# data61/stellar-random-walk

Measured on AMD Instinct MI355X. Metric: walk-steps/sec, higher is better.
Workload: dtype f64

## Files before the change

### stellar-random-walk_amd/csrc/sampler_tables.hip

```cpp
#include <cstring>

#include "engine.h"
#include "sampling.h"

namespace srw {
namespace {

constexpr int SMALL_DEG = 32;

__device__ inline bool weight_regular(float w) { return w >= 0.0f; }

struct FoStore {
  FoEnt *fo;
  __device__ inline void put(int64_t e, double cdf, int32_t id) const {
    FoEnt f; f.cdf = cdf; f.id = id; f.guide = 0; f.noff = 0; f.ndeg = 0; f.nflags = 0; fo[e] = f;
  }
  __device__ inline double cdf(int64_t e) const { return fo[e].cdf; }
  __device__ inline void set_guide(int64_t e, int32_t g) const { fo[e].guide = g; }
  __device__ inline int32_t guide(int64_t e) const { return fo[e].guide; }
};
struct SlimStore {
  double *c; int32_t *g;
  __device__ inline void put(int64_t e, double cdf, int32_t) const { c[e] = cdf; }
  __device__ inline double cdf(int64_t e) const { return c[e]; }
  __device__ inline void set_guide(int64_t e, int32_t gg) const { g[e] = gg; }
  __device__ inline int32_t guide(int64_t e) const { return g[e]; }
};

template <class ST>
__global__ void k_fo_small(Row *rows, const Ent *__restrict__ ent, ST st, int64_t n_slots) {
  for (int64_t v = blockIdx.x * (int64_t)blockDim.x + threadIdx.x; v < n_slots; v += (int64_t)gridDim.x * blockDim.x) {
    Row r = rows[v];
    if (r.deg <= 0 || r.deg > SMALL_DEG) continue;
    const Ent *row = ent + r.off;
    double sum = 0.0;
    bool irr = false;
    for (int32_t k = 0; k < r.deg; ++k) {
      float w = row[k].w;
      sum = sum + (double)w;
      irr |= !weight_regular(w);
    }
    irr |= !(sum > 0.0) || isinf(sum);
    double acc = 0.0;
    for (int32_t k = 0; k < r.deg; ++k) {
      Ent e = row[k];
      acc += (double)e.w / sum;
      st.put(r.off + k, acc, e.id);
    }
    if (irr) rows[v].flags = r.flags | ROW_IRREGULAR;
  }
}

template <class ST>
__global__ void k_fo_large(Row *rows, const Ent *__restrict__ ent, ST st, int64_t n_slots,
                           unsigned long long *next_slot) {
  const int lane = lane_id();
  while (true) {
    unsigned long long grab = 0;
    if (lane == 0) grab = atomicAdd(next_slot, 4ull);
    grab = ((unsigned long long)(uint32_t)__builtin_amdgcn_readfirstlane((int)(grab >> 32)) << 32) |
           (uint32_t)__builtin_amdgcn_readfirstlane((int)(uint32_t)grab);
    if ((int64_t)grab >= n_slots) break;
   for (int64_t v = (int64_t)grab; v < (int64_t)grab + 4 && v < n_slots; ++v) {
    Row r = rows[v];
    if (r.deg <= SMALL_DEG) continue;
    const Ent *row = ent + r.off;
    double part = 0.0;
    SumCert cert;
    bool irr = false;
    for (int32_t base = 0; base < r.deg; base += 256) {
      float wv[4]; bool ok[4];
#pragma unroll
      for (int u = 0; u < 4; ++u) {
        int32_t k = base + u * 64 + lane;
        ok[u] = k < r.deg;
        wv[u] = row[ok[u] ? k : r.deg - 1].w;
      }
#pragma unroll
      for (int u = 0; u < 4; ++u)
        if (ok[u]) { part += (double)wv[u]; cert.add(wv[u]); irr |= !weight_regular(wv[u]); }
    }
    int emin = wave_min_i32(cert.emin), emax = wave_max_i32(cert.emax);
    bool bad = __any(cert.bad);
    irr = __any(irr);
    double S;
    if (sum_is_exact(emin, emax, bad, r.deg)) {
      S = wave_sum_f64(part);
    } else {
      S = 0.0;
      for (int32_t base = 0; base < r.deg; base += 64) {
        int32_t k = base + lane;
        double wd = (k < r.deg) ? (double)row[k].w : 0.0;
        int cnt = min(64, r.deg - base);
        for (int i = 0; i < cnt; ++i) S = S + readlane_f64(wd, i);
      }
    }
    irr |= !(S > 0.0) || isinf(S);
    double acc = 0.0;
    Ent z; z.id = 0; z.w = 0.0f;
    Ent cur[4], nxt[4];
#pragma unroll
    for (int u = 0; u < 4; ++u) { int32_t k = u * 64 + lane; cur[u] = k < r.deg ? row[k] : z; }
    for (int32_t base = 0; base < r.deg; base += 256) {
#pragma unroll
      for (int u = 0; u < 4; ++u) { int64_t k = (int64_t)base + 256 + u * 64 + lane; nxt[u] = k < r.deg ? row[k] : z; }
#pragma unroll
      for (int u = 0; u < 4; ++u) {
        const int32_t cb = base + u * 64;
        if (cb < r.deg) {
          const int32_t k = cb + lane;
          const Ent e = cur[u];
          const double d = (k < r.deg) ? (double)e.w / S : 0.0;
          const int cnt = min(64, r.deg - cb);
          double mine = 0.0;
          if (cnt == 64) {
#pragma unroll
            for (int i = 0; i < 64; ++i) {
              acc = acc + readlane_f64(d, i);
              if (lane == i) mine = acc;
            }
          } else {
            for (int i = 0; i < cnt; ++i) {
              acc = acc + readlane_f64(d, i);
              if (lane == i) mine = acc;
            }
          }
          if (k < r.deg) st.put(r.off + k, mine, e.id);
        }
      }
#pragma unroll
      for (int u = 0; u < 4; ++u) cur[u] = nxt[u];
    }
    if (irr && lane == 0) rows[v].flags = r.flags | ROW_IRREGULAR;
   }
  }
}

__device__ inline double bucket_threshold(uint32_t j, uint32_t deg) {
  uint64_t m = (((uint64_t)j << 24) + deg - 1) / deg;
  return (double)m * (1.0 / 16777216.0);
}

template <class ST>
__global__ void k_guide_small(const Row *__restrict__ rows, ST st, int64_t n_slots) {
  for (int64_t v = blockIdx.x * (int64_t)blockDim.x + threadIdx.x; v < n_slots; v += (int64_t)gridDim.x * blockDim.x) {
    Row r = rows[v];
    if (r.deg <= 0 || r.deg > SMALL_DEG || (r.flags & ROW_IRREGULAR)) continue;
    int32_t k = 0;
    for (int32_t j = 0; j < r.deg; ++j) {
      double t = bucket_threshold((uint32_t)j, (uint32_t)r.deg);
      while (k < r.deg && !(st.cdf(r.off + k) >= t)) ++k;
      st.set_guide(r.off + j, k);
    }
  }
}

constexpr int GUIDE_ITEM = 8192;
struct GuideItem { uint32_t slot_lo, slot_hi_part; };

__global__ void k_guide_make_items(const Row *__restrict__ rows, int64_t n_slots, unsigned long long *counter,
                                   uint2 *__restrict__ items, unsigned long long cap) {
  for (int64_t v = blockIdx.x * (int64_t)blockDim.x + threadIdx.x; v < n_slots; v += (int64_t)gridDim.x * blockDim.x) {
    Row r = rows[v];
    if (r.deg <= SMALL_DEG || (r.flags & ROW_IRREGULAR)) continue;
    unsigned n = (unsigned)((r.deg + GUIDE_ITEM - 1) / GUIDE_ITEM);
    unsigned long long b = atomicAdd(counter, (unsigned long long)n);
    for (unsigned i = 0; i < n && b + i < cap; ++i) items[b + i] = make_uint2((uint32_t)v, ((uint32_t)(v >> 32) << 24) | i);
  }
}

template <class ST>
__device__ inline int32_t lower_bound_cdf(const ST &st, int64_t off, int32_t lo, int32_t hi, double t) {
  while (lo < hi) {
    int32_t mid = lo + ((hi - lo) >> 1);
    if (st.cdf(off + mid) >= t) hi = mid; else lo = mid + 1;
  }
  return lo;
}

template <class ST>
__global__ void k_guide_large(const Row *__restrict__ rows, ST st, const uint2 *__restrict__ items,
                              const unsigned long long *n_items_p) {
  const int lane = lane_id();
  const unsigned long long n_items = *n_items_p;
  unsigned long long wave = (blockIdx.x * (unsigned long long)blockDim.x + threadIdx.x) >> 6;
  const unsigned long long n_waves = ((unsigned long long)gridDim.x * blockDim.x) >> 6;
  for (unsigned long long it = wave; it < n_items; it += n_waves) {
    uint2 item = items[it];
    const int64_t v = (int64_t)item.x | ((int64_t)(item.y >> 24) << 32);
    const int32_t part = (int32_t)(item.y & 0xFFFFFFu);
    Row r = rows[v];
    const int32_t jb = part * GUIDE_ITEM, je = min(r.deg, jb + GUIDE_ITEM);
    int32_t start = -1;
    for (int32_t j0 = jb; j0 < je; j0 += 64) {
      const int32_t j = j0 + lane;
      int32_t ans = r.deg;
      if (j < je) {
        const double t = bucket_threshold((uint32_t)j, (uint32_t)r.deg);
        if (start < 0) {
          ans = lower_bound_cdf(st, r.off, 0, r.deg, t);
        } else {
          int32_t lo = start, step = 1;
          while (lo + step < r.deg && !(st.cdf(r.off + lo + step - 1) >= t)) { lo += step; step <<= 1; }
          ans = lower_bound_cdf(st, r.off, lo, min(r.deg, lo + step), t);
        }
        st.set_guide(r.off + j, ans);
      }
      const int last = min(63, je - j0 - 1);
      start = __builtin_amdgcn_readlane(ans, last);
    }
  }
}

__global__ void k_fo_link(const Row *__restrict__ rows, FoEnt *__restrict__ fo, int64_t n_entries, int32_t vmin,
                          int64_t n_slots) {
  for (int64_t e = blockIdx.x * (int64_t)blockDim.x + threadIdx.x; e < n_entries; e += (int64_t)gridDim.x * blockDim.x) {
    int64_t s = (int64_t)fo[e].id - vmin;
    Row r; r.off = 0; r.deg = 0; r.flags = 0;
    if (s >= 0 && s < n_slots) r = rows[s];
    fo[e].noff = r.off; fo[e].ndeg = r.deg; fo[e].nflags = r.flags;
  }
}

template <class ST>
__device__ inline void cfo_write(const ST &st, const Row *__restrict__ rows , const Ent *__restrict__ ent, int32_t vmin,
                                 int64_t n_slots, const Row &r, int32_t j, bool regular, CfoEnt *__restrict__ cfo,
                                 unsigned long long *escapes) {
  const int64_t e = r.off + j;
  const int32_t id = ent[e].id;
  const int64_t s = (int64_t)id - vmin;
  Row nr; nr.off = 0; nr.deg = 0; nr.flags = 0;
  if (s >= 0 && s < n_slots) nr = rows[s];
  bool esc = nr.deg > (int32_t)CFO_NDEG_MAX || nr.off >= ((int64_t)1 << 36);
  uint32_t cg = 0; uint32_t dbits = 0;
  if (regular) {
    const double sc = st.cdf(e) * 16777216.0;
    const uint32_t c = sc >= 16777215.0 ? 16777215u : (uint32_t)sc;
    const int32_t delta = j - st.guide(e);
    const int32_t d12 = (delta < -2047 || delta > 2047) ? CFO_GD_SAT : delta;
    dbits = (uint32_t)d12 & 0xFFFu;
    cg = c | ((dbits & 0xFFu) << 24);
  }
  CfoEnt o;
  o.cg = cg; o.id = id;
  o.link = ((uint64_t)nr.off & CFO_NOFF_MASK) | ((uint64_t)(dbits >> 8) << 36) |
           ((uint64_t)(uint32_t)min(nr.deg, (int32_t)CFO_NDEG_MAX) << 40) | ((uint64_t)((nr.flags & ROW_IRREGULAR) != 0) << 63);
  cfo[e] = o;
  if (esc) atomicAdd(escapes, 1ull);
}
template <class ST>
__global__ void k_cfo_rows(const Row *__restrict__ rows, const Row *__restrict__ link_rows, const Ent *__restrict__ ent, ST st,
                           CfoEnt *__restrict__ cfo, int64_t n_slots, int32_t vmin, unsigned long long *escapes,
                           unsigned long long *next_slot) {
  const int lane = lane_id();
  while (true) {
    unsigned long long grab = 0;
    if (lane == 0) grab = atomicAdd(next_slot, 4ull);
    grab = ((unsigned long long)(uint32_t)__builtin_amdgcn_readfirstlane((int)(grab >> 32)) << 32) |
           (uint32_t)__builtin_amdgcn_readfirstlane((int)(uint32_t)grab);
    if ((int64_t)grab >= n_slots) break;
    for (int64_t v = (int64_t)grab; v < (int64_t)grab + 4 && v < n_slots; ++v) {
      const Row r = rows[v];
      const bool regular = !(r.flags & ROW_IRREGULAR);
      for (int32_t j = lane; j < r.deg; j += 64) cfo_write(st, link_rows, ent, vmin, n_slots, r, j, regular, cfo, escapes);
    }
  }
}
__global__ void k_fo_from_slim(const Row *__restrict__ rows, const Ent *__restrict__ ent, const double *__restrict__ c,
                               const int32_t *__restrict__ g, FoEnt *__restrict__ fo, int64_t n_entries, int32_t vmin,
                               int64_t n_slots) {
  for (int64_t e = blockIdx.x * (int64_t)blockDim.x + threadIdx.x; e < n_entries; e += (int64_t)gridDim.x * blockDim.x) {
    FoEnt f; f.cdf = c[e]; f.id = ent[e].id; f.guide = g[e];
    int64_t s = (int64_t)f.id - vmin;
    Row r; r.off = 0; r.deg = 0; r.flags = 0;
    if (s >= 0 && s < n_slots) r = rows[s];
    f.noff = r.off; f.ndeg = r.deg; f.nflags = r.flags;
    fo[e] = f;
  }
}

struct PqCert {
  int emin; bool bad; double mass;
  int glsb;
  float maxv;
  __device__ PqCert() : emin(1 << 20), bad(false), mass(0.0), glsb(1 << 20), maxv(0.0f) {}
  __device__ inline void add(float x) {
    uint32_t b = __float_as_uint(x);
    int ex = (int)((b >> 23) & 0xFFu);
    if (ex == 255 || (b >> 31 && (b & 0x7FFFFFFFu))) { bad = true; return; }
    if ((b & 0x7FFFFFFFu) == 0u) return;
    int e = ex ? ex - 127 : -126;
    emin = min(emin, e);
    const uint32_t mant = (b & 0x7FFFFFu) | (ex ? 0x800000u : 0u);
    glsb = min(glsb, e - 23 + (int)__builtin_ctz(mant));
  }
  __device__ inline void add_entry(float w, float p, float q) {
    const float a = div_exact(w, q), c = div_exact(w, p);
    add(w); add(a); add(c);
    const float mx = fmaxf(w, fmaxf(a, c));
    mass += (double)mx;
    maxv = fmaxf(maxv, mx);
  }
};
__device__ inline bool pq_row_f32(int glsb, double mass) {
  if (glsb > (1 << 19) || glsb < -1000) return false;
  return mass < ldexp(1.0, 22 + glsb);
}
__device__ inline uint32_t pq_row_u16_bits(int glsb, float maxv) {
  if (glsb > 100 || glsb < -100 || !(maxv > 0.0f)) return 0u;
  const double upc = ldexp((double)maxv, -glsb);
  uint32_t c = 0;
  while (c < 7u && upc * (double)(1u << (c + 6u)) <= 65535.0) ++c;
  return (c << ROW_U16_SHIFT) | (((uint32_t)(glsb + 128) & 0xFFu) << ROW_G_SHIFT);
}
__device__ inline bool pq_row_ok(int emin, bool bad, double mass) {
  if (bad) return false;
  if (emin > (1 << 19)) return false;
  return mass <= ldexp(1.0, 51 + emin - 23);
}

__global__ void k_pq_small(Row *__restrict__ rows, const Ent *__restrict__ ent, double *__restrict__ pq,
                           uint8_t *__restrict__ ok, int64_t n_slots, float p, float q, unsigned long long *bad_rows) {
  for (int64_t v = blockIdx.x * (int64_t)blockDim.x + threadIdx.x; v < n_slots; v += (int64_t)gridDim.x * blockDim.x) {
    Row r = rows[v];
    ok[v] = 0;
    if (r.flags & ROW_PQ_BITS) { r.flags &= ~ROW_PQ_BITS; rows[v].flags = r.flags; }
    if (r.deg <= 0 || r.deg > SMALL_DEG) continue;
    PqCert c;
    for (int32_t k = 0; k < r.deg; ++k) c.add_entry(ent[r.off + k].w, p, q);
    if (!pq_row_ok(c.emin, c.bad, c.mass)) { atomicAdd(bad_rows, 1ull); continue; }
    double acc = 0.0;
    if (pq) for (int32_t k = 0; k < r.deg; ++k) { acc += (double)div_exact(ent[r.off + k].w, q); pq[r.off + k] = acc; }
    ok[v] = 1;
    rows[v].flags = r.flags | ROW_PQ_OK | (pq_row_f32(c.glsb, c.mass) ? ROW_PQ_F32 : 0u) | pq_row_u16_bits(c.glsb, c.maxv);
  }
}

__global__ void k_pq_large(Row *__restrict__ rows, const Ent *__restrict__ ent, double *__restrict__ pq,
                           uint8_t *__restrict__ ok, int64_t n_slots, float p, float q, unsigned long long *next_slot) {
  const int lane = lane_id();
  while (true) {
    unsigned long long grab = 0;
    if (lane == 0) grab = atomicAdd(next_slot, 4ull);
    grab = ((unsigned long long)(uint32_t)__builtin_amdgcn_readfirstlane((int)(grab >> 32)) << 32) |
           (uint32_t)__builtin_amdgcn_readfirstlane((int)(uint32_t)grab);
    if ((int64_t)grab >= n_slots) break;
    for (int64_t v = (int64_t)grab; v < (int64_t)grab + 4 && v < n_slots; ++v) {
      Row r = rows[v];
      if (r.deg <= SMALL_DEG) continue;
      const Ent *row = ent + r.off;
      PqCert c;
      for (int32_t k = lane; k < r.deg; k += 64) c.add_entry(row[k].w, p, q);
      const int emin = wave_min_i32(c.emin), glsb = wave_min_i32(c.glsb);
      const bool bad = __any(c.bad);
      const double mass = wave_sum_f64(bad ? 0.0 : c.mass);
      const float maxv = __int_as_float(wave_max_i32(__float_as_int(bad ? 0.0f : c.maxv)));
      if (!pq_row_ok(emin, bad, mass)) { if (lane == 0) atomicAdd(next_slot + 1, 1ull); continue; }
      double carry = 0.0;
      for (int32_t base = 0; base < r.deg; base += 64) {
        int32_t k = base + lane;
        double x = k < r.deg ? (double)div_exact(row[k].w, q) : 0.0;
        for (int o = 1; o < 64; o <<= 1) { double t = __shfl_up(x, o); if (lane >= o) x += t; }
        if (pq && k < r.deg) pq[r.off + k] = carry + x;
        carry += readlane_f64(x, 63);
      }
      if (lane == 0) { ok[v] = 1; rows[v].flags = r.flags | ROW_PQ_OK | (pq_row_f32(glsb, mass) ? ROW_PQ_F32 : 0u) | pq_row_u16_bits(glsb, maxv); }
    }
  }
}

}

void build_pq_tables(srw_handle *h, float p, float q) {
  Graph &g = h->g;
  uint32_t pb, qb; memcpy(&pb, &p, 4); memcpy(&qb, &q, 4);
  if (g.has_pq && g.pq_pbits == pb && g.pq_qbits == qb) return;
  hipStream_t st = h->stream;
  g.has_pq = false;
  size_t free_b = 0, total_b = 0;
  SRW_HIP(hipMemGetInfo(&free_b, &total_b));
  const bool unit = !getenv("SRW_NO_UNIT_PQ") && graph_has_unit_weights(h);
  g.pq_unit = unit ? (double)(1.0f / q) : 0.0;
  const size_t need = (unit ? 0 : (size_t)g.n_entries * sizeof(double)) + (size_t)g.n_slots;
  if (!unit && g.pq.n < (size_t)g.n_entries && free_b < need + ((size_t)8 << 30)) return;
  if (unit) g.pq.release(); else g.pq.ensure((size_t)g.n_entries);
  g.pq_ok.ensure((size_t)g.n_slots);
  int gs = (int)std::min<int64_t>(std::max<int64_t>((g.n_slots + 255) / 256, 1), 256 * 32);
  DevBuf<unsigned long long> next_slot; next_slot.alloc(2);
  SRW_HIP(hipMemsetAsync(next_slot.p, 0, 16, st));
  hipLaunchKernelGGL(k_pq_small, dim3(gs), dim3(256), 0, st, g.rows.p, g.ent.p, g.pq.p, g.pq_ok.p, g.n_slots, p, q, next_slot.p + 1);
  hipLaunchKernelGGL(k_pq_large, dim3(256 * 8), dim3(256), 0, st, g.rows.p, g.ent.p, g.pq.p, g.pq_ok.p, g.n_slots, p, q,
                     next_slot.p);
  SRW_HIP(hipGetLastError());
  unsigned long long nbad = 0;
  SRW_HIP(hipMemcpyAsync(&nbad, next_slot.p + 1, 8, hipMemcpyDeviceToHost, st));
  SRW_HIP(hipStreamSynchronize(st));
  g.pq_bad_rows = (int64_t)nbad;
  g.pq_pbits = pb; g.pq_qbits = qb; g.has_pq = true;
}

template <class ST>
static void run_cdf_and_guide(srw_handle *h, ST st, DevBuf<uint2> &items, DevBuf<unsigned long long> &n_items) {
  Graph &g = h->g;
  hipStream_t stq = h->stream;
  int64_t tb = (g.n_slots + 255) / 256;
  int gs = (int)std::min<int64_t>(std::max<int64_t>(tb, 1), 256 * 32);
  DevBuf<unsigned long long> next_slot; next_slot.alloc(1);
  SRW_HIP(hipMemsetAsync(next_slot.p, 0, 8, stq));
  hipLaunchKernelGGL((k_fo_small<ST>), dim3(gs), dim3(256), 0, stq, g.rows.p, g.ent.p, st, g.n_slots);
  hipLaunchKernelGGL((k_fo_large<ST>), dim3(256 * 8), dim3(256), 0, stq, g.rows.p, g.ent.p, st, g.n_slots, next_slot.p);
  hipLaunchKernelGGL((k_guide_small<ST>), dim3(gs), dim3(256), 0, stq, g.rows.p, st, g.n_slots);
  const unsigned long long cap = (unsigned long long)g.n_entries / SMALL_DEG + 1024;
  items.alloc((size_t)cap); n_items.alloc(2);
  SRW_HIP(hipMemsetAsync(n_items.p, 0, 16, stq));
  hipLaunchKernelGGL(k_guide_make_items, dim3(gs), dim3(256), 0, stq, g.rows.p, g.n_slots, n_items.p, items.p, cap);
  hipLaunchKernelGGL((k_guide_large<ST>), dim3(256 * 16), dim3(256), 0, stq, g.rows.p, st, items.p, n_items.p);
  SRW_HIP(hipGetLastError());
  SRW_HIP(hipStreamSynchronize(stq));
}

template <class ST>
static unsigned long long run_cfo(srw_handle *h, ST st, unsigned long long *esc_word, const Row *link_rows = nullptr) {
  Graph &g = h->g;
  hipStream_t stq = h->stream;
  DevBuf<unsigned long long> next_slot; next_slot.alloc(1);
  SRW_HIP(hipMemsetAsync(next_slot.p, 0, 8, stq));
  SRW_HIP(hipMemsetAsync(esc_word, 0, 8, stq));
  hipLaunchKernelGGL((k_cfo_rows<ST>), dim3(256 * 8), dim3(256), 0, stq, g.rows.p, link_rows ? link_rows : g.rows.p, g.ent.p, st,
                     g.cfo.p, g.n_slots, g.vmin, esc_word, next_slot.p);
  unsigned long long n_esc = 0;
  SRW_HIP(hipMemcpyAsync(&n_esc, esc_word, 8, hipMemcpyDeviceToHost, stq));
  SRW_HIP(hipStreamSynchronize(stq));
  SRW_HIP(hipGetLastError());
  return n_esc;
}

void build_first_order_tables(srw_handle *h, bool want_exact) {
  Graph &g = h->g;
  const bool sharded = h->cfg.world > 1;
  if (g.has_cfo_local && !sharded) { g.has_cfo = true; g.has_cfo_local = false; }
  if (want_exact ? g.has_fo : (g.has_cfo || sharded || g.cfo_rejected || g.n_entries == 0) && (g.has_cfo || g.has_fo)) return;
  hipStream_t st = h->stream;
  DevBuf<uint2> items; DevBuf<unsigned long long> n_items;
  if (!want_exact && g.has_fo) {
    n_items.alloc(2);
    g.cfo.alloc((size_t)g.n_entries);
    if (run_cfo(h, FoStore{g.fo.p}, n_items.p + 1) == 0) g.has_cfo = true;
    else { g.cfo.release(); g.cfo_rejected = true; }
    return;
  }
  if (!want_exact && !sharded && g.n_entries > 0 && !g.cfo_rejected) {
    DevBuf<double> c; DevBuf<int32_t> gd;
    c.alloc((size_t)g.n_entries); gd.alloc((size_t)g.n_entries);
    SlimStore slim{c.p, gd.p};
    run_cdf_and_guide(h, slim, items, n_items);
    g.cfo.alloc((size_t)g.n_entries);
    if (getenv("SRW_TIMING")) fprintf(stderr, "[timing] compact first-order table: %zu bytes at %p\n", (size_t)g.n_entries * sizeof(CfoEnt), (void *)g.cfo.p);
    if (run_cfo(h, slim, n_items.p + 1) == 0) { g.has_cfo = true; return; }
    g.cfo.release(); g.cfo_rejected = true;
    g.fo.alloc((size_t)g.n_entries);
    int ge = (int)std::min<int64_t>((g.n_entries + 255) / 256, 256 * 32);
    hipLaunchKernelGGL(k_fo_from_slim, dim3(ge), dim3(256), 0, st, g.rows.p, g.ent.p, c.p, gd.p, g.fo.p, g.n_entries, g.vmin,
                       g.n_slots);
    SRW_HIP(hipGetLastError());
    SRW_HIP(hipStreamSynchronize(st));
    g.has_fo = true;
    return;
  }
  g.fo.alloc((size_t)g.n_entries);
  FoStore fs{g.fo.p};
  run_cdf_and_guide(h, fs, items, n_items);
  if (g.n_entries > 0) {
    int ge = (int)std::min<int64_t>((g.n_entries + 255) / 256, 256 * 32);
    hipLaunchKernelGGL(k_fo_link, dim3(ge), dim3(256), 0, st, g.rows.p, g.fo.p, g.n_entries, g.vmin, g.n_slots);
  }
  SRW_HIP(hipGetLastError());
  SRW_HIP(hipStreamSynchronize(st));
  g.has_fo = true;
}

bool build_local_cfo(srw_handle *h) {
  Graph &g = h->g;
  if (g.has_cfo || g.cfo_linked || g.has_cfo_local) return true;
  if (g.cfo_rejected || g.n_entries == 0) return false;
  build_first_order_tables(h, true);
  DevBuf<unsigned long long> esc; esc.alloc(1);
  g.cfo.alloc((size_t)g.n_entries);
  if (run_cfo(h, FoStore{g.fo.p}, esc.p) != 0) { g.cfo.release(); g.cfo_rejected = true; return false; }
  g.has_cfo_local = true;
  return true;
}

namespace {
__global__ void k_rows_max(unsigned long long *__restrict__ acc, const unsigned long long *__restrict__ other, int64_t n_words) {
  for (int64_t i = blockIdx.x * (int64_t)blockDim.x + threadIdx.x; i < n_words; i += (int64_t)gridDim.x * blockDim.x) {
    const long long a = (long long)acc[i], b = (long long)other[i];
    acc[i] = (unsigned long long)(a > b ? a : b);
  }
}
__global__ void k_rows_unlinkable(const Row *__restrict__ rows, int64_t n_slots, unsigned long long *count) {
  for (int64_t i = blockIdx.x * (int64_t)blockDim.x + threadIdx.x; i < n_slots; i += (int64_t)gridDim.x * blockDim.x) {
    const Row r = rows[i];
    if (r.deg > (int32_t)CFO_NDEG_MAX || r.off >= ((int64_t)1 << 36)) atomicAdd(count, 1ull);
  }
}
}

void shard_rows_export(srw_handle *h, void *d_rows, int64_t n_slots) {
  Graph &g = h->g;
  if (!g.loaded) throw Error(SRW_ERR_INVALID, "no graph loaded");
  if (n_slots != g.n_slots) throw Error(SRW_ERR_INVALID, "row table size mismatch");
  build_first_order_tables(h, true);
  SRW_HIP(hipMemcpyAsync(d_rows, g.rows.p, (size_t)n_slots * sizeof(Row), hipMemcpyDeviceToDevice, h->stream));
  SRW_HIP(hipStreamSynchronize(h->stream));
}

void shard_rows_merge(srw_handle *h, void *d_rows, const void *d_other, int64_t n_slots) {
  if (n_slots != h->g.n_slots) throw Error(SRW_ERR_INVALID, "row table size mismatch");
  const int64_t n_words = n_slots * 2;
  const int blocks = (int)std::min<int64_t>(std::max<int64_t>((n_words + 255) / 256, 1), 256 * 32);
  hipLaunchKernelGGL(k_rows_max, dim3(blocks), dim3(256), 0, h->stream, (unsigned long long *)d_rows, (const unsigned long long *)d_other, n_words);
  SRW_HIP(hipGetLastError());
  SRW_HIP(hipStreamSynchronize(h->stream));
}

bool shard_rows_commit(srw_handle *h, const void *d_rows_all, int64_t n_slots) {
  Graph &g = h->g;
  if (!g.loaded) throw Error(SRW_ERR_INVALID, "no graph loaded");
  if (n_slots != g.n_slots) throw Error(SRW_ERR_INVALID, "row table size mismatch");
  build_first_order_tables(h, true);
  shard_rows_release(h);
  if (g.has_cfo_local && h->cfg.world == 1) { g.has_cfo = true; g.has_cfo_local = false; }
  if (g.has_cfo_local) { g.cfo.release(); g.has_cfo_local = false; }
  g.rows_all.alloc((size_t)n_slots);
  SRW_HIP(hipMemcpyAsync(g.rows_all.p, d_rows_all, (size_t)n_slots * sizeof(Row), hipMemcpyDeviceToDevice, h->stream));
  if (g.n_entries == 0) { SRW_HIP(hipStreamSynchronize(h->stream)); g.cfo_linked = true; return true; }
  DevBuf<unsigned long long> esc; esc.alloc(1);
  {
    unsigned long long n_bad = 0;
    SRW_HIP(hipMemsetAsync(esc.p, 0, 8, h->stream));
    const int blocks = (int)std::min<int64_t>(std::max<int64_t>((n_slots + 255) / 256, 1), 256 * 32);
    hipLaunchKernelGGL(k_rows_unlinkable, dim3(blocks), dim3(256), 0, h->stream, g.rows_all.p, n_slots, esc.p);
    SRW_HIP(hipGetLastError());
    SRW_HIP(hipMemcpyAsync(&n_bad, esc.p, 8, hipMemcpyDeviceToHost, h->stream));
    SRW_HIP(hipStreamSynchronize(h->stream));
    if (n_bad != 0) { g.rows_all.release(); return false; }
  }
  if (g.has_cfo) {
    if (h->cfg.world != 1) throw Error(SRW_ERR_INVALID, "srw_shard_rows_commit: the handle already holds an unsharded compact table");
    SRW_HIP(hipStreamSynchronize(h->stream)); g.cfo_linked = true; return true;
  }
  g.cfo.alloc((size_t)g.n_entries);
  if (run_cfo(h, FoStore{g.fo.p}, esc.p, g.rows_all.p) != 0) { g.cfo.release(); g.rows_all.release(); return false; }
  g.cfo_linked = true;
  return true;
}

void shard_rows_release(srw_handle *h) {
  Graph &g = h->g;
  if (g.cfo_linked && !g.has_cfo) g.cfo.release();
  g.cfo_linked = false;
  g.rows_all.release();
}

}
```

Before: 39.85 billion.

## Restructure first-order table build into degree-sorted work lists with split partial sums

Replaces the atomic slot-grabbing kernels that build first-order CDF/guide tables with precomputed work lists. Large rows are bucketed by degree class and split into 8192-entry parts whose sums are computed in parallel before a per-row chain pass. Small rows get a fused kernel that computes CDF and guide in one pass and writes directly to the compact or full table. This targets load imbalance and extra passes in table construction, at the cost of a host sync for counts, more kernels and extra scratch buffers. The walk-step rate only changes if the table build is counted in the timed region.

```diff
diff --git a/stellar-random-walk_amd/csrc/sampler_tables.hip b/stellar-random-walk_amd/csrc/sampler_tables.hip
--- a/stellar-random-walk_amd/csrc/sampler_tables.hip
+++ b/stellar-random-walk_amd/csrc/sampler_tables.hip
@@ -27,11 +27,29 @@
   __device__ inline int32_t guide(int64_t e) const { return g[e]; }
 };
 
-template <class ST>
-__global__ void k_fo_small(Row *rows, const Ent *__restrict__ ent, ST st, int64_t n_slots) {
-  for (int64_t v = blockIdx.x * (int64_t)blockDim.x + threadIdx.x; v < n_slots; v += (int64_t)gridDim.x * blockDim.x) {
+constexpr int PART = 8192;
+enum { CTR_CLASS = 0, CTR_ITEMS = 32, CTR_CURSOR = 33, CTR_ESC = 66, CTR_WORDS = 68 };
+struct ClassBases { uint32_t b[32]; };
+struct alignas(8) PartSum { double sum; int32_t emin, emax; uint32_t fl, pad; };
+
+__device__ inline int deg_class(int32_t deg) { return 31 - __clz(deg); }
+__device__ inline uint32_t n_parts(int32_t deg) { return ((uint32_t)deg + PART - 1) / PART; }
+__device__ inline int32_t part_end(int32_t deg, int32_t kb) { return deg - kb > PART ? kb + PART : deg; }
+__device__ inline void block_range(int64_t n, int64_t &lo, int64_t &hi) {
+  const int64_t per = (n + gridDim.x - 1) / gridDim.x;
+  lo = blockIdx.x * per; hi = min(n, lo + per);
+}
+
+__global__ void k_rows_prepare(Row *rows, const Ent *__restrict__ ent, int64_t n_slots, int flag_small,
+                               unsigned long long *ctr) {
+  __shared__ unsigned s_cnt[33];
+  if (threadIdx.x < 33) s_cnt[threadIdx.x] = 0;
+  __syncthreads();
+  int64_t lo, hi; block_range(n_slots, lo, hi);
+  for (int64_t v = lo + threadIdx.x; v < hi; v += blockDim.x) {
     Row r = rows[v];
-    if (r.deg <= 0 || r.deg > SMALL_DEG) continue;
+    if (r.deg > SMALL_DEG) { atomicAdd(&s_cnt[deg_class(r.deg)], 1u); atomicAdd(&s_cnt[32], n_parts(r.deg)); continue; }
+    if (!flag_small || r.deg <= 0) continue;
     const Ent *row = ent + r.off;
     double sum = 0.0;
     bool irr = false;
@@ -41,48 +59,96 @@
       irr |= !weight_regular(w);
     }
     irr |= !(sum > 0.0) || isinf(sum);
-    double acc = 0.0;
-    for (int32_t k = 0; k < r.deg; ++k) {
-      Ent e = row[k];
-      acc += (double)e.w / sum;
-      st.put(r.off + k, acc, e.id);
-    }
     if (irr) rows[v].flags = r.flags | ROW_IRREGULAR;
   }
-}
-
-template <class ST>
-__global__ void k_fo_large(Row *rows, const Ent *__restrict__ ent, ST st, int64_t n_slots,
-                           unsigned long long *next_slot) {
+  __syncthreads();
+  if (threadIdx.x < 33 && s_cnt[threadIdx.x]) atomicAdd(&ctr[CTR_CLASS + threadIdx.x], (unsigned long long)s_cnt[threadIdx.x]);
+}
+
+__global__ void k_rows_scatter(const Row *__restrict__ rows, int64_t n_slots, ClassBases bases, unsigned long long *ctr,
+                               uint2 *__restrict__ large, uint32_t n_large, uint2 *__restrict__ items, uint32_t n_items) {
+  __shared__ unsigned s_cnt[33], s_base[33];
+  if (threadIdx.x < 33) s_cnt[threadIdx.x] = 0;
+  __syncthreads();
+  int64_t lo, hi; block_range(n_slots, lo, hi);
+  for (int64_t v = lo + threadIdx.x; v < hi; v += blockDim.x) {
+    const int32_t deg = rows[v].deg;
+    if (deg > SMALL_DEG) { atomicAdd(&s_cnt[deg_class(deg)], 1u); atomicAdd(&s_cnt[32], n_parts(deg)); }
+  }
+  __syncthreads();
+  if (threadIdx.x < 33) {
+    const unsigned c = s_cnt[threadIdx.x];
+    const unsigned long long got = c ? atomicAdd(&ctr[CTR_CURSOR + threadIdx.x], (unsigned long long)c) : 0ull;
+    s_base[threadIdx.x] = (threadIdx.x < 32 ? bases.b[threadIdx.x] : 0u) + (unsigned)got;
+    s_cnt[threadIdx.x] = 0;
+  }
+  __syncthreads();
+  for (int64_t v = lo + threadIdx.x; v < hi; v += blockDim.x) {
+    const int32_t deg = rows[v].deg;
+    if (deg <= SMALL_DEG) continue;
+    const int cls = deg_class(deg);
+    const uint32_t n = n_parts(deg);
+    const uint32_t pos = s_base[cls] + atomicAdd(&s_cnt[cls], 1u);
+    const uint32_t ib = s_base[32] + atomicAdd(&s_cnt[32], n);
+    if (pos >= n_large || ib > n_items || n > n_items - ib) continue;
+    large[pos] = make_uint2((uint32_t)v, ib);
+    for (uint32_t i = 0; i < n; ++i) items[ib + i] = make_uint2((uint32_t)v, i);
+  }
+}
+
+__device__ inline uint32_t wave_index() { return uni((uint32_t)((blockIdx.x * blockDim.x + threadIdx.x) >> 6)); }
+__device__ inline uint32_t wave_count() { return (uint32_t)((gridDim.x * blockDim.x) >> 6); }
+
+__global__ void k_fo_sum_parts(const Row *__restrict__ rows, const Ent *__restrict__ ent, const uint2 *__restrict__ items,
+                               uint32_t n_items, PartSum *__restrict__ parts) {
   const int lane = lane_id();
-  while (true) {
-    unsigned long long grab = 0;
-    if (lane == 0) grab = atomicAdd(next_slot, 4ull);
-    grab = ((unsigned long long)(uint32_t)__builtin_amdgcn_readfirstlane((int)(grab >> 32)) << 32) |
-           (uint32_t)__builtin_amdgcn_readfirstlane((int)(uint32_t)grab);
-    if ((int64_t)grab >= n_slots) break;
-   for (int64_t v = (int64_t)grab; v < (int64_t)grab + 4 && v < n_slots; ++v) {
-    Row r = rows[v];
-    if (r.deg <= SMALL_DEG) continue;
+  for (uint32_t it = wave_index(); it < n_items; it += wave_count()) {
+    const uint2 item = items[it];
+    const Row r = rows[item.x];
     const Ent *row = ent + r.off;
+    const int32_t kb = (int32_t)item.y * PART, ke = part_end(r.deg, kb);
     double part = 0.0;
     SumCert cert;
     bool irr = false;
-    for (int32_t base = 0; base < r.deg; base += 256) {
+    for (int32_t base = kb; base < ke; base += 256) {
       float wv[4]; bool ok[4];
 #pragma unroll
       for (int u = 0; u < 4; ++u) {
         int32_t k = base + u * 64 + lane;
-        ok[u] = k < r.deg;
-        wv[u] = row[ok[u] ? k : r.deg - 1].w;
+        ok[u] = k < ke;
+        wv[u] = row[ok[u] ? k : ke - 1].w;
       }
 #pragma unroll
       for (int u = 0; u < 4; ++u)
         if (ok[u]) { part += (double)wv[u]; cert.add(wv[u]); irr |= !weight_regular(wv[u]); }
     }
-    int emin = wave_min_i32(cert.emin), emax = wave_max_i32(cert.emax);
-    bool bad = __any(cert.bad);
+    const int emin = wave_min_i32(cert.emin), emax = wave_max_i32(cert.emax);
+    const bool bad = __any(cert.bad);
     irr = __any(irr);
+    part = wave_sum_f64(part);
+    if (lane == 0) { PartSum p; p.sum = part; p.emin = emin; p.emax = emax; p.fl = (bad ? 1u : 0u) | (irr ? 2u : 0u); p.pad = 0; parts[it] = p; }
+  }
+}
+
+template <class ST>
+__global__ void k_fo_chain(Row *rows, const Ent *__restrict__ ent, ST st, const uint2 *__restrict__ large, uint32_t n_large,
+                           const PartSum *__restrict__ parts) {
+  const int lane = lane_id();
+  for (uint32_t li = wave_index(); li < n_large; li += wave_count()) {
+    const uint2 le = large[li];
+    const int64_t v = (int64_t)le.x;
+    Row r = rows[v];
+    const Ent *row = ent + r.off;
+    double part = 0.0;
+    int emin = 1 << 20, emax = -(1 << 20);
+    uint32_t fl = 0;
+    for (uint32_t i = (uint32_t)lane, n = n_parts(r.deg); i < n; i += 64) {
+      const PartSum p = parts[le.y + i];
+      part += p.sum; emin = min(emin, p.emin); emax = max(emax, p.emax); fl |= p.fl;
+    }
+    emin = wave_min_i32(emin); emax = wave_max_i32(emax);
+    const bool bad = __any(fl & 1u);
+    bool irr = __any(fl & 2u);
     double S;
     if (sum_is_exact(emin, emax, bad, r.deg)) {
       S = wave_sum_f64(part);
@@ -132,7 +198,6 @@
       for (int u = 0; u < 4; ++u) cur[u] = nxt[u];
     }
     if (irr && lane == 0) rows[v].flags = r.flags | ROW_IRREGULAR;
-   }
   }
 }
 
@@ -141,33 +206,7 @@
   return (double)m * (1.0 / 16777216.0);
 }
 
-template <class ST>
-__global__ void k_guide_small(const Row *__restrict__ rows, ST st, int64_t n_slots) {
-  for (int64_t v = blockIdx.x * (int64_t)blockDim.x + threadIdx.x; v < n_slots; v += (int64_t)gridDim.x * blockDim.x) {
-    Row r = rows[v];
-    if (r.deg <= 0 || r.deg > SMALL_DEG || (r.flags & ROW_IRREGULAR)) continue;
-    int32_t k = 0;
-    for (int32_t j = 0; j < r.deg; ++j) {
-      double t = bucket_threshold((uint32_t)j, (uint32_t)r.deg);
-      while (k < r.deg && !(st.cdf(r.off + k) >= t)) ++k;
-      st.set_guide(r.off + j, k);
-    }
-  }
-}
-
-constexpr int GUIDE_ITEM = 8192;
-struct GuideItem { uint32_t slot_lo, slot_hi_part; };
-
-__global__ void k_guide_make_items(const Row *__restrict__ rows, int64_t n_slots, unsigned long long *counter,
-                                   uint2 *__restrict__ items, unsigned long long cap) {
-  for (int64_t v = blockIdx.x * (int64_t)blockDim.x + threadIdx.x; v < n_slots; v += (int64_t)gridDim.x * blockDim.x) {
-    Row r = rows[v];
-    if (r.deg <= SMALL_DEG || (r.flags & ROW_IRREGULAR)) continue;
-    unsigned n = (unsigned)((r.deg + GUIDE_ITEM - 1) / GUIDE_ITEM);
-    unsigned long long b = atomicAdd(counter, (unsigned long long)n);
-    for (unsigned i = 0; i < n && b + i < cap; ++i) items[b + i] = make_uint2((uint32_t)v, ((uint32_t)(v >> 32) << 24) | i);
-  }
-}
+constexpr int GUIDE_ITEM = PART;
 
 template <class ST>
 __device__ inline int32_t lower_bound_cdf(const ST &st, int64_t off, int32_t lo, int32_t hi, double t) {
@@ -179,18 +218,13 @@
 }
 
 template <class ST>
-__global__ void k_guide_large(const Row *__restrict__ rows, ST st, const uint2 *__restrict__ items,
-                              const unsigned long long *n_items_p) {
+__global__ void k_guide_large(const Row *__restrict__ rows, ST st, const uint2 *__restrict__ items, uint32_t n_items) {
   const int lane = lane_id();
-  const unsigned long long n_items = *n_items_p;
-  unsigned long long wave = (blockIdx.x * (unsigned long long)blockDim.x + threadIdx.x) >> 6;
-  const unsigned long long n_waves = ((unsigned long long)gridDim.x * blockDim.x) >> 6;
-  for (unsigned long long it = wave; it < n_items; it += n_waves) {
-    uint2 item = items[it];
-    const int64_t v = (int64_t)item.x | ((int64_t)(item.y >> 24) << 32);
-    const int32_t part = (int32_t)(item.y & 0xFFFFFFu);
-    Row r = rows[v];
-    const int32_t jb = part * GUIDE_ITEM, je = min(r.deg, jb + GUIDE_ITEM);
+  for (uint32_t it = wave_index(); it < n_items; it += wave_count()) {
+    const uint2 item = items[it];
+    const Row r = rows[item.x];
+    if (r.flags & ROW_IRREGULAR) continue;
+    const int32_t jb = (int32_t)item.y * GUIDE_ITEM, je = part_end(r.deg, jb);
     int32_t start = -1;
     for (int32_t j0 = jb; j0 < je; j0 += 64) {
       const int32_t j = j0 + lane;
@@ -222,21 +256,14 @@
   }
 }
 
-template <class ST>
-__device__ inline void cfo_write(const ST &st, const Row *__restrict__ rows , const Ent *__restrict__ ent, int32_t vmin,
-                                 int64_t n_slots, const Row &r, int32_t j, bool regular, CfoEnt *__restrict__ cfo,
-                                 unsigned long long *escapes) {
-  const int64_t e = r.off + j;
-  const int32_t id = ent[e].id;
-  const int64_t s = (int64_t)id - vmin;
-  Row nr; nr.off = 0; nr.deg = 0; nr.flags = 0;
-  if (s >= 0 && s < n_slots) nr = rows[s];
+__device__ inline void cfo_put(CfoEnt *__restrict__ cfo, int64_t e, int32_t j, int32_t id, const Row &nr, bool regular, double cdf,
+                               int32_t guide, unsigned long long *escapes) {
   bool esc = nr.deg > (int32_t)CFO_NDEG_MAX || nr.off >= ((int64_t)1 << 36);
   uint32_t cg = 0; uint32_t dbits = 0;
   if (regular) {
-    const double sc = st.cdf(e) * 16777216.0;
+    const double sc = cdf * 16777216.0;
     const uint32_t c = sc >= 16777215.0 ? 16777215u : (uint32_t)sc;
-    const int32_t delta = j - st.guide(e);
+    const int32_t delta = j - guide;
     const int32_t d12 = (delta < -2047 || delta > 2047) ? CFO_GD_SAT : delta;
     dbits = (uint32_t)d12 & 0xFFFu;
     cg = c | ((dbits & 0xFFu) << 24);
@@ -248,34 +275,100 @@
   cfo[e] = o;
   if (esc) atomicAdd(escapes, 1ull);
 }
-template <class ST>
-__global__ void k_cfo_rows(const Row *__restrict__ rows, const Row *__restrict__ link_rows, const Ent *__restrict__ ent, ST st,
-                           CfoEnt *__restrict__ cfo, int64_t n_slots, int32_t vmin, unsigned long long *escapes,
-                           unsigned long long *next_slot) {
+__device__ inline Row link_row(const Row *__restrict__ rows, int32_t id, int32_t vmin, int64_t n_slots) {
+  const int64_t s = (int64_t)id - vmin;
+  Row nr; nr.off = 0; nr.deg = 0; nr.flags = 0;
+  if (s >= 0 && s < n_slots) nr = rows[s];
+  return nr;
+}
+template <class ST>
+__device__ inline void cfo_write(const ST &st, const Row *__restrict__ rows , const Ent *__restrict__ ent, int32_t vmin,
+                                 int64_t n_slots, const Row &r, int32_t j, bool regular, CfoEnt *__restrict__ cfo,
+                                 unsigned long long *escapes) {
+  const int64_t e = r.off + j;
+  const int32_t id = ent[e].id;
+  const Row nr = link_row(rows, id, vmin, n_slots);
+  cfo_put(cfo, e, j, id, nr, regular, regular ? st.cdf(e) : 0.0, regular ? st.guide(e) : 0, escapes);
+}
+
+struct FoSink {
+  FoEnt *fo;
+  __device__ inline void emit(const Row &r, int32_t j, int32_t id, bool regular, double cdf, int32_t guide) const {
+    FoEnt f; f.cdf = cdf; f.id = id; f.guide = guide; f.noff = 0; f.ndeg = 0; f.nflags = 0; fo[r.off + j] = f;
+  }
+};
+struct CfoSink {
+  CfoEnt *cfo; const Row *link_rows; int32_t vmin; int64_t n_slots; unsigned long long *escapes;
+  __device__ inline void emit(const Row &r, int32_t j, int32_t id, bool regular, double cdf, int32_t guide) const {
+    cfo_put(cfo, r.off + j, j, id, link_row(link_rows, id, vmin, n_slots), regular, cdf, guide, escapes);
+  }
+};
+
+template <class SINK>
+__global__ void k_small_rows(const Row *__restrict__ rows, const Ent *__restrict__ ent, SINK sink, int64_t n_slots) {
+  for (int64_t v = blockIdx.x * (int64_t)blockDim.x + threadIdx.x; v < n_slots; v += (int64_t)gridDim.x * blockDim.x) {
+    const Row r = rows[v];
+    if (r.deg <= 0 || r.deg > SMALL_DEG) continue;
+    const Ent *row = ent + r.off;
+    const bool regular = !(r.flags & ROW_IRREGULAR);
+    double sum = 0.0;
+    for (int32_t k = 0; k < r.deg; ++k) sum = sum + (double)row[k].w;
+    double acc = 0.0, acc_k = 0.0;
+    acc_k += (double)row[0].w / sum;
+    int32_t k = 0;
+    for (int32_t j = 0; j < r.deg; ++j) {
+      const Ent e = row[j];
+      acc += (double)e.w / sum;
+      int32_t guide = 0;
+      if (regular) {
+        const double t = bucket_threshold((uint32_t)j, (uint32_t)r.deg);
+        while (k < r.deg && !(acc_k >= t)) {
+          ++k;
+          if (k < r.deg) acc_k += (double)row[k].w / sum;
+        }
+        guide = k;
+      }
+      sink.emit(r, j, e.id, regular, acc, guide);
+    }
+  }
+}
+
+template <class ST>
+__global__ void k_cfo_small(const Row *__restrict__ rows, const Row *__restrict__ link_rows, const Ent *__restrict__ ent, ST st,
+                            CfoEnt *__restrict__ cfo, int64_t n_slots, int32_t vmin, unsigned long long *escapes) {
+  for (int64_t v = blockIdx.x * (int64_t)blockDim.x + threadIdx.x; v < n_slots; v += (int64_t)gridDim.x * blockDim.x) {
+    const Row r = rows[v];
+    if (r.deg <= 0 || r.deg > SMALL_DEG) continue;
+    const bool regular = !(r.flags & ROW_IRREGULAR);
+    for (int32_t j = 0; j < r.deg; ++j) cfo_write(st, link_rows, ent, vmin, n_slots, r, j, regular, cfo, escapes);
+  }
+}
+template <class ST>
+__global__ void k_cfo_items(const Row *__restrict__ rows, const Row *__restrict__ link_rows, const Ent *__restrict__ ent, ST st,
+                            CfoEnt *__restrict__ cfo, int64_t n_slots, int32_t vmin, unsigned long long *escapes,
+                            const uint2 *__restrict__ items, uint32_t n_items) {
   const int lane = lane_id();
-  while (true) {
-    unsigned long long grab = 0;
-    if (lane == 0) grab = atomicAdd(next_slot, 4ull);
-    grab = ((unsigned long long)(uint32_t)__builtin_amdgcn_readfirstlane((int)(grab >> 32)) << 32) |
-           (uint32_t)__builtin_amdgcn_readfirstlane((int)(uint32_t)grab);
-    if ((int64_t)grab >= n_slots) break;
-    for (int64_t v = (int64_t)grab; v < (int64_t)grab + 4 && v < n_slots; ++v) {
-      const Row r = rows[v];
-      const bool regular = !(r.flags & ROW_IRREGULAR);
-      for (int32_t j = lane; j < r.deg; j += 64) cfo_write(st, link_rows, ent, vmin, n_slots, r, j, regular, cfo, escapes);
-    }
-  }
-}
-__global__ void k_fo_from_slim(const Row *__restrict__ rows, const Ent *__restrict__ ent, const double *__restrict__ c,
-                               const int32_t *__restrict__ g, FoEnt *__restrict__ fo, int64_t n_entries, int32_t vmin,
-                               int64_t n_slots) {
-  for (int64_t e = blockIdx.x * (int64_t)blockDim.x + threadIdx.x; e < n_entries; e += (int64_t)gridDim.x * blockDim.x) {
-    FoEnt f; f.cdf = c[e]; f.id = ent[e].id; f.guide = g[e];
-    int64_t s = (int64_t)f.id - vmin;
-    Row r; r.off = 0; r.deg = 0; r.flags = 0;
-    if (s >= 0 && s < n_slots) r = rows[s];
-    f.noff = r.off; f.ndeg = r.deg; f.nflags = r.flags;
-    fo[e] = f;
+  for (uint32_t it = wave_index(); it < n_items; it += wave_count()) {
+    const uint2 item = items[it];
+    const Row r = rows[item.x];
+    const bool regular = !(r.flags & ROW_IRREGULAR);
+    const int32_t jb = (int32_t)item.y * PART, je = part_end(r.deg, jb);
+    for (int32_t j = jb + lane; j < je; j += 64) cfo_write(st, link_rows, ent, vmin, n_slots, r, j, regular, cfo, escapes);
+  }
+}
+__global__ void k_fo_from_slim(const uint2 *__restrict__ items, uint32_t n_items, const Row *__restrict__ rows, const Ent *__restrict__ ent,
+                               const double *__restrict__ c, const int32_t *__restrict__ g, FoEnt *__restrict__ fo) {
+  const int lane = lane_id();
+  for (uint32_t it = wave_index(); it < n_items; it += wave_count()) {
+    const uint2 item = items[it];
+    const Row r = rows[item.x];
+    const bool regular = !(r.flags & ROW_IRREGULAR);
+    const int32_t jb = (int32_t)item.y * PART, je = part_end(r.deg, jb);
+    for (int32_t j = jb + lane; j < je; j += 64) {
+      const int64_t e = r.off + j;
+      FoEnt f; f.cdf = c[e]; f.id = ent[e].id; f.guide = regular ? g[e] : 0; f.noff = 0; f.ndeg = 0; f.nflags = 0;
+      fo[e] = f;
+    }
   }
 }
 
@@ -399,40 +492,82 @@
   g.pq_pbits = pb; g.pq_qbits = qb; g.has_pq = true;
 }
 
-template <class ST>
-static void run_cdf_and_guide(srw_handle *h, ST st, DevBuf<uint2> &items, DevBuf<unsigned long long> &n_items) {
+struct WorkLists {
+  DevBuf<unsigned long long> ctr, buf;
+  uint2 *large = nullptr, *items = nullptr;
+  PartSum *parts = nullptr;
+  uint32_t n_large = 0, n_items = 0;
+  unsigned long long *escapes() const { return ctr.p + CTR_ESC; }
+};
+static int slot_grid(int64_t n_slots) { return (int)std::min<int64_t>(std::max<int64_t>((n_slots + 255) / 256, 1), 256 * 32); }
+static int wave_grid(uint32_t n_waves) { return (int)std::min<uint32_t>(std::max<uint32_t>((n_waves + 3) / 4, 1), 256 * 16); }
+
+static void build_work_lists(srw_handle *h, WorkLists &wl, bool flag_small) {
   Graph &g = h->g;
   hipStream_t stq = h->stream;
-  int64_t tb = (g.n_slots + 255) / 256;
-  int gs = (int)std::min<int64_t>(std::max<int64_t>(tb, 1), 256 * 32);
-  DevBuf<unsigned long long> next_slot; next_slot.alloc(1);
-  SRW_HIP(hipMemsetAsync(next_slot.p, 0, 8, stq));
-  hipLaunchKernelGGL((k_fo_small<ST>), dim3(gs), dim3(256), 0, stq, g.rows.p, g.ent.p, st, g.n_slots);
-  hipLaunchKernelGGL((k_fo_large<ST>), dim3(256 * 8), dim3(256), 0, stq, g.rows.p, g.ent.p, st, g.n_slots, next_slot.p);
-  hipLaunchKernelGGL((k_guide_small<ST>), dim3(gs), dim3(256), 0, stq, g.rows.p, st, g.n_slots);
-  const unsigned long long cap = (unsigned long long)g.n_entries / SMALL_DEG + 1024;
-  items.alloc((size_t)cap); n_items.alloc(2);
-  SRW_HIP(hipMemsetAsync(n_items.p, 0, 16, stq));
-  hipLaunchKernelGGL(k_guide_make_items, dim3(gs), dim3(256), 0, stq, g.rows.p, g.n_slots, n_items.p, items.p, cap);
-  hipLaunchKernelGGL((k_guide_large<ST>), dim3(256 * 16), dim3(256), 0, stq, g.rows.p, st, items.p, n_items.p);
+  if (g.n_slots > ((int64_t)1 << 32)) throw Error(SRW_ERR_INVALID, "first-order tables: more than 2^32 id slots");
+  const int gb = (int)std::min<int64_t>(std::max<int64_t>((g.n_slots + 4095) / 4096, 1), 2048);
+  wl.ctr.alloc(CTR_WORDS);
+  SRW_HIP(hipMemsetAsync(wl.ctr.p, 0, CTR_WORDS * sizeof(unsigned long long), stq));
+  hipLaunchKernelGGL(k_rows_prepare, dim3(gb), dim3(256), 0, stq, g.rows.p, g.ent.p, g.n_slots, flag_small ? 1 : 0, wl.ctr.p);
   SRW_HIP(hipGetLastError());
+  unsigned long long cnt[33];
+  SRW_HIP(hipMemcpyAsync(cnt, wl.ctr.p, sizeof cnt, hipMemcpyDeviceToHost, stq));
   SRW_HIP(hipStreamSynchronize(stq));
-}
-
-template <class ST>
-static unsigned long long run_cfo(srw_handle *h, ST st, unsigned long long *esc_word, const Row *link_rows = nullptr) {
+  ClassBases bases;
+  unsigned long long pos = 0;
+  for (int c = 31; c >= 0; --c) { bases.b[c] = (uint32_t)pos; pos += cnt[c]; }
+  if (pos >= (1ull << 32) || cnt[32] >= (1ull << 32)) throw Error(SRW_ERR_INVALID, "first-order tables: too many large rows");
+  wl.n_large = (uint32_t)pos; wl.n_items = (uint32_t)cnt[32];
+  if (wl.n_large == 0) return;
+  wl.buf.alloc((size_t)wl.n_large + (size_t)wl.n_items * (flag_small ? 4 : 1));
+  wl.large = (uint2 *)wl.buf.p;
+  wl.items = wl.large + wl.n_large;
+  wl.parts = flag_small ? (PartSum *)(wl.items + wl.n_items) : nullptr;
+  hipLaunchKernelGGL(k_rows_scatter, dim3(gb), dim3(256), 0, stq, g.rows.p, g.n_slots, bases, wl.ctr.p, wl.large, wl.n_large, wl.items,
+                     wl.n_items);
+  SRW_HIP(hipGetLastError());
+}
+
+template <class ST>
+static void run_cdf_and_guide(srw_handle *h, ST st, WorkLists &wl) {
   Graph &g = h->g;
   hipStream_t stq = h->stream;
-  DevBuf<unsigned long long> next_slot; next_slot.alloc(1);
-  SRW_HIP(hipMemsetAsync(next_slot.p, 0, 8, stq));
-  SRW_HIP(hipMemsetAsync(esc_word, 0, 8, stq));
-  hipLaunchKernelGGL((k_cfo_rows<ST>), dim3(256 * 8), dim3(256), 0, stq, g.rows.p, link_rows ? link_rows : g.rows.p, g.ent.p, st,
-                     g.cfo.p, g.n_slots, g.vmin, esc_word, next_slot.p);
+  build_work_lists(h, wl, true);
+  if (wl.n_large == 0) return;
+  hipLaunchKernelGGL(k_fo_sum_parts, dim3(wave_grid(wl.n_items)), dim3(256), 0, stq, g.rows.p, g.ent.p, wl.items, wl.n_items, wl.parts);
+  hipLaunchKernelGGL((k_fo_chain<ST>), dim3(wave_grid(std::min<uint32_t>(wl.n_large, 256 * 8 * 4))), dim3(256), 0, stq, g.rows.p, g.ent.p, st,
+                     wl.large, wl.n_large, wl.parts);
+  hipLaunchKernelGGL((k_guide_large<ST>), dim3(wave_grid(wl.n_items)), dim3(256), 0, stq, g.rows.p, st, wl.items, wl.n_items);
+  SRW_HIP(hipGetLastError());
+}
+
+template <class ST>
+static unsigned long long run_cfo(srw_handle *h, ST st, WorkLists &wl, bool store_has_small, const Row *link_rows = nullptr) {
+  Graph &g = h->g;
+  hipStream_t stq = h->stream;
+  if (!link_rows) link_rows = g.rows.p;
+  unsigned long long *esc = wl.escapes();
+  SRW_HIP(hipMemsetAsync(esc, 0, 8, stq));
+  if (store_has_small)
+    hipLaunchKernelGGL((k_cfo_small<ST>), dim3(slot_grid(g.n_slots)), dim3(256), 0, stq, g.rows.p, link_rows, g.ent.p, st, g.cfo.p, g.n_slots,
+                       g.vmin, esc);
+  else
+    hipLaunchKernelGGL((k_small_rows<CfoSink>), dim3(slot_grid(g.n_slots)), dim3(256), 0, stq, g.rows.p, g.ent.p,
+                       CfoSink{g.cfo.p, link_rows, g.vmin, g.n_slots, esc}, g.n_slots);
+  if (wl.n_large)
+    hipLaunchKernelGGL((k_cfo_items<ST>), dim3(wave_grid(wl.n_items)), dim3(256), 0, stq, g.rows.p, link_rows, g.ent.p, st, g.cfo.p, g.n_slots,
+                       g.vmin, esc, wl.items, wl.n_items);
+  SRW_HIP(hipGetLastError());
   unsigned long long n_esc = 0;
-  SRW_HIP(hipMemcpyAsync(&n_esc, esc_word, 8, hipMemcpyDeviceToHost, stq));
+  SRW_HIP(hipMemcpyAsync(&n_esc, esc, 8, hipMemcpyDeviceToHost, stq));
   SRW_HIP(hipStreamSynchronize(stq));
-  SRW_HIP(hipGetLastError());
   return n_esc;
+}
+static unsigned long long run_cfo_from_exact(srw_handle *h, const Row *link_rows = nullptr) {
+  WorkLists wl;
+  build_work_lists(h, wl, false);
+  return run_cfo(h, FoStore{h->g.fo.p}, wl, true, link_rows);
 }
 
 void build_first_order_tables(srw_handle *h, bool want_exact) {
@@ -441,39 +576,31 @@
   if (g.has_cfo_local && !sharded) { g.has_cfo = true; g.has_cfo_local = false; }
   if (want_exact ? g.has_fo : (g.has_cfo || sharded || g.cfo_rejected || g.n_entries == 0) && (g.has_cfo || g.has_fo)) return;
   hipStream_t st = h->stream;
-  DevBuf<uint2> items; DevBuf<unsigned long long> n_items;
   if (!want_exact && g.has_fo) {
-    n_items.alloc(2);
     g.cfo.alloc((size_t)g.n_entries);
-    if (run_cfo(h, FoStore{g.fo.p}, n_items.p + 1) == 0) g.has_cfo = true;
+    if (run_cfo_from_exact(h) == 0) g.has_cfo = true;
     else { g.cfo.release(); g.cfo_rejected = true; }
     return;
   }
+  WorkLists wl;
+  const int ge = (int)std::min<int64_t>(std::max<int64_t>((g.n_entries + 255) / 256, 1), 256 * 32);
   if (!want_exact && !sharded && g.n_entries > 0 && !g.cfo_rejected) {
     DevBuf<double> c; DevBuf<int32_t> gd;
     c.alloc((size_t)g.n_entries); gd.alloc((size_t)g.n_entries);
     SlimStore slim{c.p, gd.p};
-    run_cdf_and_guide(h, slim, items, n_items);
+    run_cdf_and_guide(h, slim, wl);
     g.cfo.alloc((size_t)g.n_entries);
     if (getenv("SRW_TIMING")) fprintf(stderr, "[timing] compact first-order table: %zu bytes at %p\n", (size_t)g.n_entries * sizeof(CfoEnt), (void *)g.cfo.p);
-    if (run_cfo(h, slim, n_items.p + 1) == 0) { g.has_cfo = true; return; }
+    if (run_cfo(h, slim, wl, false) == 0) { g.has_cfo = true; return; }
     g.cfo.release(); g.cfo_rejected = true;
     g.fo.alloc((size_t)g.n_entries);
-    int ge = (int)std::min<int64_t>((g.n_entries + 255) / 256, 256 * 32);
-    hipLaunchKernelGGL(k_fo_from_slim, dim3(ge), dim3(256), 0, st, g.rows.p, g.ent.p, c.p, gd.p, g.fo.p, g.n_entries, g.vmin,
-                       g.n_slots);
-    SRW_HIP(hipGetLastError());
-    SRW_HIP(hipStreamSynchronize(st));
-    g.has_fo = true;
-    return;
-  }
-  g.fo.alloc((size_t)g.n_entries);
-  FoStore fs{g.fo.p};
-  run_cdf_and_guide(h, fs, items, n_items);
-  if (g.n_entries > 0) {
-    int ge = (int)std::min<int64_t>((g.n_entries + 255) / 256, 256 * 32);
-    hipLaunchKernelGGL(k_fo_link, dim3(ge), dim3(256), 0, st, g.rows.p, g.fo.p, g.n_entries, g.vmin, g.n_slots);
-  }
+    hipLaunchKernelGGL(k_fo_from_slim, dim3(ge), dim3(256), 0, st, wl.items, wl.n_items, g.rows.p, g.ent.p, c.p, gd.p, g.fo.p);
+  } else {
+    g.fo.alloc((size_t)g.n_entries);
+    run_cdf_and_guide(h, FoStore{g.fo.p}, wl);
+  }
+  hipLaunchKernelGGL((k_small_rows<FoSink>), dim3(slot_grid(g.n_slots)), dim3(256), 0, st, g.rows.p, g.ent.p, FoSink{g.fo.p}, g.n_slots);
+  if (g.n_entries > 0) hipLaunchKernelGGL(k_fo_link, dim3(ge), dim3(256), 0, st, g.rows.p, g.fo.p, g.n_entries, g.vmin, g.n_slots);
   SRW_HIP(hipGetLastError());
   SRW_HIP(hipStreamSynchronize(st));
   g.has_fo = true;
@@ -484,9 +611,8 @@
   if (g.has_cfo || g.cfo_linked || g.has_cfo_local) return true;
   if (g.cfo_rejected || g.n_entries == 0) return false;
   build_first_order_tables(h, true);
-  DevBuf<unsigned long long> esc; esc.alloc(1);
   g.cfo.alloc((size_t)g.n_entries);
-  if (run_cfo(h, FoStore{g.fo.p}, esc.p) != 0) { g.cfo.release(); g.cfo_rejected = true; return false; }
+  if (run_cfo_from_exact(h) != 0) { g.cfo.release(); g.cfo_rejected = true; return false; }
   g.has_cfo_local = true;
   return true;
 }
@@ -551,7 +677,7 @@
     SRW_HIP(hipStreamSynchronize(h->stream)); g.cfo_linked = true; return true;
   }
   g.cfo.alloc((size_t)g.n_entries);
-  if (run_cfo(h, FoStore{g.fo.p}, esc.p, g.rows_all.p) != 0) { g.cfo.release(); g.rows_all.release(); return false; }
+  if (run_cfo_from_exact(h, g.rows_all.p) != 0) { g.cfo.release(); g.rows_all.release(); return false; }
   g.cfo_linked = true;
   return true;
 }
```

After: 36.75 billion. -7.8%, worse.
